# JiaweiXu8/AD-GS

Measured on AMD Instinct MI355X. Metric: fwd+bwd frames/s, higher is better.
Workload: dtype f32; 1 GPU; C3: 1000000 Gaussians, 1920x1280, SH deg 3, 8 dynamic objects, flow+semantic outputs, 1 camera/GPU/step; P=1000000, camera_pool=16 cameras / time stamps per GPU, cycled one per step (train.py:55-61), settle_steps=75, capacity_reruns=0, launch=eager, parallelism=single GPU, gradient_exchange=none, camera_streams=1

## Files before the change

ad-gs_amd/csrc/api.hip:

```cpp
#include "common.h"
#include "kernels.h"
#include "../../include/adgs_rasterizer.h"
#include "../../include/adgs_optim.h"

#include <atomic>
#include <chrono>
#include <mutex>
#include <vector>
#include <cstdlib>
#include <algorithm>
#include <cmath>
#include <cstring>

namespace adgs {

static thread_local std::string g_last_error;
struct FrameContext {
	adgs_frame_stats stats;
	size_t hint_cells, hint_fine;
	unsigned hint_max_cell_chunks;
	bool bucket_frame_pending;
	long long reruns;
	int last_order_hint;
	uint32_t* slab_bounds;
// ... 36 lines not shown
constexpr size_t IMG_HEADER_WORDS = 16;
struct ImgState {
	uint32_t* header; uint32_t* n_contrib; uint2* ranges;
	static ImgState carve(char* chunk, size_t npix, size_t ntiles, size_t* bytes) {
		Carver c(chunk); ImgState s;
		s.header = c.take<uint32_t>(IMG_HEADER_WORDS);
		s.n_contrib = c.take<uint32_t>(npix);
		s.ranges = c.take<uint2>(ntiles);
		if (bytes) *bytes = c.size();
		return s;
	}
};
struct BinState {
	uint64_t* keys_unsorted; uint64_t* keys; uint32_t* list_unsorted; uint32_t* list; char* sort_temp;
	static BinState carve(char* chunk, size_t R, size_t* bytes) {
		Carver c(chunk); BinState b;
		b.list = c.take<uint32_t>(R);
		b.list_unsorted = c.take<uint32_t>(R);
		b.keys = c.take<uint64_t>(R);
		b.keys_unsorted = c.take<uint64_t>(R);
		b.sort_temp = c.take<char>(sort_temp_bytes(R));
		if (bytes) *bytes = c.size();
		return b;
	}
};

struct GeomStateV2 {
	Splat* splats; uint8_t* clamped; uint32_t* cells_touched; uint32_t* offsets; uint32_t* fine_touched; uint4* dupinfo;
	float* gacc; float* sh0; char* scan_temp; unsigned long long* fine_total;
	float* ddir;
	uint32_t* counters; uint32_t* cell_start; uint2* cell_work; uint32_t* bounds; uint32_t* counts;
	static constexpr size_t COUNTER_WORDS = MAX_CELLS + 2 * SCAN_AUX_SLOTS + 8;
	uint32_t* cell_count() const { return counters; }
	unsigned long long* bucket_fine_total() const { return reinterpret_cast<unsigned long long*>(counters + MAX_CELLS); }
	uint32_t* d_counts() const { return counters + MAX_CELLS + 2 * SCAN_AUX_SLOTS; }
	static GeomStateV2 carve(char* chunk, size_t P, size_t* bytes, bool with_ddir, size_t ncells = 0) {
		Carver c(chunk); GeomStateV2 g;
		g.counters = c.take<uint32_t>(COUNTER_WORDS);
		g.cell_start = c.take<uint32_t>(MAX_CELLS + 1);
		g.cell_work = c.take<uint2>(MAX_CELLS + 1);
		g.splats = c.take<Splat>(P);
		g.gacc = c.take<float>(P * GACC_STRIDE);
		g.dupinfo = c.take<uint4>(P);
		g.clamped = c.take<uint8_t>(P);
		g.cells_touched = c.take<uint32_t>(P + 1);
		g.offsets = c.take<uint32_t>(P + 1);
		g.fine_touched = c.take<uint32_t>(P + 1);
		g.sh0 = c.take<float>(P * 3);
		g.fine_total = c.take<unsigned long long>(SCAN_AUX_SLOTS);
		g.scan_temp = c.take<char>(scan_temp_bytes(P + 1));
		g.ddir = with_ddir ? c.take<float>(P * 9) : nullptr;
		const size_t nc = std::min<size_t>(ncells, (size_t)MAX_CELLS + 1);
		g.bounds = c.take<uint32_t>(nc * SLAB_ROW);
		g.counts = c.take<uint32_t>(((P + 255) / 256) * nc);
		if (bytes) *bytes = c.size();
		return g;
	}
};
struct ImgStateV2 {
	uint32_t* header; uint32_t* n_contrib; uint2* cell_ranges; uint32_t* tile_last_chunk; uint32_t* tile_consumed; uint32_t* tile_order; uint32_t* tile_scanned; uint32_t* tile_batches;
	static ImgStateV2 carve(char* chunk, size_t npix, size_t ntiles, size_t ncells, size_t* bytes) {
		Carver c(chunk); ImgStateV2 s;
		s.header = c.take<uint32_t>(IMG_HEADER_WORDS);
		s.n_contrib = c.take<uint32_t>(npix);
		s.cell_ranges = c.take<uint2>(ncells);
		s.tile_last_chunk = c.take<uint32_t>(ntiles);
		s.tile_consumed = c.take<uint32_t>(ntiles);
		s.tile_order = c.take<uint32_t>(ntiles);
		s.tile_scanned = c.take<uint32_t>(ntiles);
		s.tile_batches = c.take<uint32_t>(ntiles);
		if (bytes) *bytes = c.size();
		return s;
	}
};
struct BinStateV2 {
	uint32_t* pool_cursor; uint32_t* pool;
	uint64_t* keys_unsorted; uint64_t* keys; uint32_t* list_unsorted; uint32_t* list; char* sort_temp;
	uint32_t* rec_key; uint2* rec_im; uint2* entries; uint32_t* slow_list;
	static size_t slab_grid(size_t R_cells, size_t ncells) { return std::max<size_t>(2 * R_cells / SLAB_TARGET_FOREIGN + ncells + 1, ncells << forced_lg()); }
	static int forced_lg() { const char* v = getenv("ADGS_SLABS_LG"); return (v && *v) ? std::min(std::max(atoi(v), 0), (int)MAX_SLAB_LG) : 0; }
	static size_t pool_chunks(size_t R_fine, size_t ntiles) { return R_fine / WAVE + (2 * (size_t)POOL_BLOCK + 1) * ntiles + 1; }
	static BinStateV2 carve_buckets(char* chunk, size_t R_cells, size_t R_fine, size_t ntiles, size_t* bytes, size_t ncells = 0) {
		Carver c(chunk); BinStateV2 b;
		b.pool_cursor = c.take<uint32_t>(64);
		b.pool = c.take<uint32_t>(pool_chunks(R_fine, ntiles) * CHUNK_WORDS);
		b.entries = c.take<uint2>(R_cells + 1);
		b.rec_im = c.take<uint2>(R_cells);
		b.rec_key = c.take<uint32_t>(R_cells);
		b.slow_list = c.take<uint32_t>(1 + slab_grid(R_cells, ncells));
		b.keys = nullptr; b.keys_unsorted = nullptr; b.sort_temp = nullptr; b.list = nullptr; b.list_unsorted = nullptr;
		if (bytes) *bytes = c.size();
		return b;
	}
	static BinStateV2 carve(char* chunk, size_t R_cells, size_t R_fine, size_t ntiles, size_t* bytes) {
		Carver c(chunk); BinStateV2 b;
		b.pool_cursor = c.take<uint32_t>(64);
		b.pool = c.take<uint32_t>(pool_chunks(R_fine, ntiles) * CHUNK_WORDS);
		b.list = c.take<uint32_t>(R_cells);
		b.list_unsorted = c.take<uint32_t>(R_cells);
		b.keys = c.take<uint64_t>(R_cells);
		b.keys_unsorted = c.take<uint64_t>(R_cells);
		b.sort_temp = c.take<char>(sort_temp_bytes(R_cells));
		b.rec_key = nullptr; b.rec_im = nullptr; b.entries = nullptr; b.slow_list = nullptr;
		if (bytes) *bytes = c.size();
		return b;
	}
};
// ... 1193 lines not shown
```

ad-gs_amd/csrc/binning.hip:

```cpp
#include "common.h"
#include "kernels.h"

namespace adgs {
namespace {

constexpr int CS_THREADS = MAX_CELLS;
constexpr int GS_THREADS = 512, GS_WAVES = GS_THREADS / WAVE, GS_ITEMS = GS_NMAX / GS_THREADS;

__device__ __forceinline__ uint32_t wave_incl_scan_u32(uint32_t v, int lane) {
#pragma unroll
	for (int off = 1; off < WAVE; off <<= 1) { const uint32_t o = __shfl_up(v, off, WAVE); if (lane >= off) v += o; }
	return v;
}

__device__ __forceinline__ uint32_t block_excl_scan_1024(uint32_t v, uint32_t* s_wave , uint32_t* total) {
	const int tid = threadIdx.x, lane = tid & (WAVE - 1), wid = tid / WAVE;
	const uint32_t incl = wave_incl_scan_u32(v, lane);
	__syncthreads();
	if (lane == WAVE - 1) s_wave[wid] = incl;
	__syncthreads();
	uint32_t off = 0, tot = 0;
#pragma unroll
	for (int w = 0; w < CS_THREADS / WAVE; w++) { const uint32_t x = s_wave[w]; if (w < wid) off += x; tot += x; }
	*total = tot;
	return off + incl - v;
}

__global__ void __launch_bounds__(256) bin_prepare_kernel(FramePrologue p) { run_frame_prologue(p); }

__global__ void __launch_bounds__(256) cell_colscan_kernel(uint32_t* __restrict__ counts, int nblocks, int ncells, uint32_t* __restrict__ cell_count) {
	__shared__ uint32_t s_w[256 / WAVE];
	__shared__ uint32_t s_carry;
	const int c = blockIdx.x, tid = threadIdx.x, lane = tid & (WAVE - 1), wid = tid / WAVE;
	if (tid == 0) s_carry = 0u;
	__syncthreads();
	for (int b0 = 0; b0 < nblocks; b0 += 256 * 8) {
		uint32_t v[8], sum = 0;
#pragma unroll
		for (int k = 0; k < 8; k++) v[k] = counts[(size_t)min(b0 + tid * 8 + k, nblocks - 1) * ncells + c];
#pragma unroll
		for (int k = 0; k < 8; k++) { if (b0 + tid * 8 + k >= nblocks) v[k] = 0u; sum += v[k]; }
		const uint32_t incl = wave_incl_scan_u32(sum, lane);
		if (lane == WAVE - 1) s_w[wid] = incl;
		__syncthreads();
		uint32_t off = s_carry, tot = 0;
#pragma unroll
		for (int w = 0; w < 256 / WAVE; w++) { const uint32_t x = s_w[w]; if (w < wid) off += x; tot += x; }
		uint32_t run = off + incl - sum;
#pragma unroll
		for (int k = 0; k < 8; k++) { const int b = b0 + tid * 8 + k; if (b < nblocks) counts[(size_t)b * ncells + c] = run; run += v[k]; }
		__syncthreads();
		if (tid == 0) s_carry += tot;
		__syncthreads();
	}
	if (tid == 0) cell_count[c] = s_carry;
}

__global__ void __launch_bounds__(CS_THREADS) cell_scan_kernel(CellScanArgs a) {
	__shared__ uint32_t s_wave[CS_THREADS / WAVE];
	const int c = threadIdx.x;
	uint32_t n = 0;
	if (c < a.ncells) n = a.cell_count[c];
	uint32_t total, nchunks_total, work_total;
	const uint32_t start = block_excl_scan_1024(n, s_wave, &total);
	const uint32_t nch = (n + GS_NMAX - 1) / GS_NMAX;
	(void)block_excl_scan_1024(nch, s_wave, &nchunks_total);
	uint32_t lg = 0;
	while (lg < (uint32_t)MAX_SLAB_LG && (n >> lg) > a.slab_target) lg++;
	if (a.force_lg >= 0) lg = min((uint32_t)a.force_lg, (uint32_t)MAX_SLAB_LG);
	const uint32_t m = (c < a.ncells && n) ? 1u << lg : 0u;
	const uint32_t w0 = block_excl_scan_1024(m, s_wave, &work_total);
	if (c < a.ncells) { a.cell_start[c] = start; a.cell_ranges[c] = make_uint2(start, start + n); a.cell_work[c] = make_uint2(w0, lg); }
	if (c == 0) {
		a.cell_start[a.ncells] = total; a.cell_work[a.ncells] = make_uint2(work_total, 0u);
		const uint32_t over = nchunks_total > a.max_chunks ? 1u : 0u;
		unsigned long long fine = 0ull;
		for (int k = 0; k < SCAN_AUX_SLOTS; k++) fine += a.fine_total[k];
		const uint32_t nofit = (over || total > a.cap_cells || fine > a.cap_fine) ? 1u : 0u;
		a.d_counts[0] = total; a.d_counts[1] = work_total; a.d_counts[2] = over; a.d_counts[3] = nofit;
		a.d_counts[4] = 0u; a.d_counts[5] = 0u;
		a.d_counts[6] = (uint32_t)fine; a.d_counts[7] = (uint32_t)(fine >> 32);
		if (a.box) {
			a.box->r_cells = total; a.box->r_fine = fine; a.box->oversize = over; a.box->n_groups = nchunks_total; a.box->overflow = nofit;
			if (nofit) a.box->overflow_count = a.box->overflow_count + 1u;
			a.box->cap_cells = a.cap_cells; a.box->cap_fine = a.cap_fine;
			__threadfence_system();
			a.box->seq = a.seq;
		}
	}
}

__global__ void __launch_bounds__(256) cell_scatter_kernel(int P, const uint4* __restrict__ dupinfo, const uint32_t* __restrict__ cell_start,
	const uint32_t* __restrict__ counts, uint32_t* __restrict__ rec_key, uint2* __restrict__ rec_im, uint32_t cap, int cell_tiles, int cgx, int ncells, uint32_t* __restrict__ pool_cursor, uint32_t* __restrict__ slow_list) {
	__shared__ uint32_t s_cnt[MAX_CELLS];
	__shared__ uint32_t s_base[MAX_CELLS];
	const int idx = blockIdx.x * blockDim.x + threadIdx.x;
	if (idx == 0) { *pool_cursor = 0u; slow_list[0] = 0u; }
	const uint4 d = dupinfo[min(idx, P - 1)];
	for (int c = threadIdx.x; c < ncells; c += 256) { s_cnt[c] = 0u; s_base[c] = cell_start[c] + counts[(size_t)blockIdx.x * ncells + c]; }
	__syncthreads();
	if (idx >= P) return;
	const uint32_t minx = d.x & 0xFFFFu, miny = d.x >> 16, maxx = d.y & 0xFFFFu, maxy = d.y >> 16;
	if (maxx <= minx || maxy <= miny) return;
	const uint32_t c0x = minx / cell_tiles, c1x = (maxx - 1) / cell_tiles, c0y = miny / cell_tiles, c1y = (maxy - 1) / cell_tiles;
	for (uint32_t y = c0y; y <= c1y; y++)
		for (uint32_t x = c0x; x <= c1x; x++) {
			const uint32_t c = y * cgx + x;
			const uint32_t pos = s_base[c] + atomicAdd(s_cnt + c, 1u);
			const uint32_t ty0 = y * cell_tiles, tx0 = x * cell_tiles;
			const uint32_t r0 = max(miny, ty0) - ty0, r1 = min(maxy, ty0 + cell_tiles) - ty0;
			const uint32_t q0 = max(minx, tx0) - tx0, q1 = min(maxx, tx0 + cell_tiles) - tx0;
			const uint32_t rows = ((1u << r1) - 1u) & ~((1u << r0) - 1u), cols = ((1u << q1) - 1u) & ~((1u << q0) - 1u);
			if (pos < cap) { rec_key[pos] = d.z; rec_im[pos] = make_uint2((uint32_t)idx, rows | (cols << cell_tiles)); }
		}
}

__device__ __forceinline__ uint32_t slab128_of(const uint32_t* row , uint32_t key) {
	const uint32_t q = (row[31] <= key ? 1u : 0u) + (row[63] <= key ? 1u : 0u) + (row[95] <= key ? 1u : 0u);
	uint32_t r = 0;
#pragma unroll
	for (int i = 0; i < 8; i++) {
		const uint4 v = *reinterpret_cast<const uint4*>(row + 32 * q + 4 * i);
		r += (v.x <= key ? 1u : 0u) + (v.y <= key ? 1u : 0u) + (v.z <= key ? 1u : 0u) + ((i < 7 && v.w <= key) ? 1u : 0u);
	}
	return 32u * q + r;
}

__device__ __forceinline__ void publish_bound(uint32_t* __restrict__ bounds_out, uint32_t cell, uint32_t r, uint32_t n, uint32_t key) {
	const uint32_t j = (uint32_t)(((unsigned long long)r * (unsigned)SLAB_ROW + n - 1ull) / n);
	if (j >= 1u && j < (uint32_t)SLAB_ROW && (uint32_t)(((unsigned long long)j * n) / (unsigned)SLAB_ROW) == r) bounds_out[(size_t)cell * SLAB_ROW + j - 1u] = key;
}

struct SlabLds {
	uint32_t a[GS_NMAX];
	uint32_t b[GS_NMAX];
	uint32_t c[GS_NMAX];
	uint32_t cc[256];
	uint32_t red[3 * GS_WAVES];
	uint32_t row[SLAB_ROW];
	unsigned long long stack[72];
	uint32_t nsel, below, last;
};
static_assert(GS_WAVES * 256 <= GS_NMAX, "the radix sort's per-wave digit counters live in SlabLds::c");

constexpr int BS_NB = GS_NMAX, BS_NC = 256, BS_BMAX = 32;
__device__ __forceinline__ bool bucket_rank(SlabLds& s, uint32_t n, const uint32_t (&key)[GS_ITEMS], const uint32_t (&id)[GS_ITEMS], uint32_t (&rank)[GS_ITEMS]) {
	const int tid = threadIdx.x, lane = tid & (WAVE - 1), wid = tid / WAVE;
	uint32_t fb[GS_ITEMS], arr[GS_ITEMS];
	uint32_t kmin = 0xffffffffu, kmax = 0u;
#pragma unroll
	for (int r = 0; r < GS_ITEMS; r++) if ((uint32_t)(r * GS_THREADS + tid) < n) { kmin = min(kmin, key[r]); kmax = max(kmax, key[r]); }
	__syncthreads();
// ... 203 lines not shown
#pragma unroll
	for (int r = 0; r < GS_ITEMS; r++) {
		const uint32_t i = r * GS_THREADS + tid;
		id[r] = i; src[r] = 0u;
		key[r] = a.rec_key[range.x + min((uint32_t)(((unsigned long long)(2u * i + 1u) * n_c) / (2ull * S)), n_c - 1u)];
	}
	bool radix = false;
	if (!bucket_rank(s, S, key, id, rank)) { radix = true; radix_rank(s, S, key, id, src, rank); }
#pragma unroll
	for (int r = 0; r < GS_ITEMS; r++) {
		const bool have = radix ? rank[r] != 0xffffffffu : (uint32_t)(r * GS_THREADS + tid) < S;
		if (have) publish_bound(bounds, cell, rank[r], S, key[r]);
	}
}

__global__ void __launch_bounds__(GS_THREADS, 6) slab_sort_kernel(SlabSortArgs a) {
	__shared__ __attribute__((aligned(16))) SlabLds s;
	const int tid = threadIdx.x, lane = tid & (WAVE - 1);
	if (!(a.d_counts[2] == 0u && a.d_counts[3] == 0u && a.d_counts[0] <= a.cap) || blockIdx.x >= a.d_counts[1]) return;
	for (int i = tid; i <= a.ncells; i += GS_THREADS) {
		const uint2 cwv = a.cell_work[i], rg = a.cell_ranges[min(i, a.ncells - 1)];
		s.a[i] = cwv.x; s.b[i] = cwv.y; s.c[2 * i] = rg.x; s.c[2 * i + 1] = rg.y;
	}
	__syncthreads();
	uint32_t cell = 0;
	{
		uint32_t len = (uint32_t)a.ncells;
		uint32_t lo_i = 0;
		while (len > 0u) { const uint32_t half = len >> 1; if (s.a[lo_i + half] <= blockIdx.x) { lo_i += half + 1u; len -= half + 1u; } else len = half; }
		cell = lo_i - 1u;
	}
	const uint32_t lg = s.b[cell], slab = blockIdx.x - s.a[cell];
	const int shift = MAX_SLAB_LG - (int)lg;
	const uint2 range = make_uint2(s.c[2 * cell], s.c[2 * cell + 1]);
	__syncthreads();
	const uint32_t n_c = range.y - range.x;
	if (n_c == 0u || slab >= (1u << lg)) return;
	uint32_t lo = 0u, hi = 0u; bool open_top = true, sorted = true;
	if (lg > 0u) {
		const uint32_t* row = a.bounds + (size_t)cell * SLAB_ROW;
		const uint32_t w0 = row[min(lane, 126)], w1 = row[min(lane + 1, 126)], w2 = row[min(lane + 64, 126)], w3 = row[min(lane + 65, 126)];
		sorted = __ballot((lane < 126 && w0 > w1) || (lane + 64 < 126 && w2 > w3)) == 0ull;
		if (slab > 0u) lo = row[(slab << shift) - 1u];
		open_top = slab == (1u << lg) - 1u;
		if (!open_top) hi = row[((slab + 1u) << shift) - 1u];
	}
	if (tid == 0) { s.nsel = 0u; s.below = 0u; }
	__syncthreads();
	uint32_t my_below = 0;
	if (sorted) {
		const uint32_t off = range.x & 3u, n_el = off + n_c;
		const uint4* __restrict__ kw = reinterpret_cast<const uint4*>(a.rec_key + (range.x - off));
		const uint32_t n_w = (n_el + 3u) >> 2;
		const uint64_t lt = (lane == 0) ? 0ull : (~0ull >> (WAVE - lane));
		constexpr int SW = 8;
		for (uint32_t wbase = 0; wbase < n_w; wbase += GS_THREADS * SW) {
			uint4 kq[SW];
#pragma unroll
			for (int u = 0; u < SW; u++) kq[u] = kw[min(wbase + u * GS_THREADS + tid, n_w - 1u)];
			uint32_t selbits = 0, wave_n = 0;
#pragma unroll
			for (int u = 0; u < SW; u++) {
				const uint32_t kk[4] = { kq[u].x, kq[u].y, kq[u].z, kq[u].w };
#pragma unroll
				for (int e = 0; e < 4; e++) {
					const uint32_t el = (wbase + u * GS_THREADS + tid) * 4u + e;
					const bool have = el >= off && el < n_el, sel = have && kk[e] >= lo && (open_top || kk[e] < hi);
					my_below += (have && kk[e] < lo) ? 1u : 0u;
					selbits |= sel ? 1u << (4 * u + e) : 0u;
					wave_n += (uint32_t)__popcll(__ballot(sel));
				}
			}
			if (wave_n != 0u) {
				uint32_t at0 = 0;
				if (lane == 0) at0 = atomicAdd(&s.nsel, wave_n);
				at0 = __shfl(at0, 0, WAVE);
				uint32_t run = 0;
#pragma unroll
				for (int u = 0; u < SW; u++) {
					const uint32_t kk[4] = { kq[u].x, kq[u].y, kq[u].z, kq[u].w };
#pragma unroll
					for (int e = 0; e < 4; e++) {
						const bool sel = (selbits >> (4 * u + e)) & 1u;
						const uint64_t m = __ballot(sel);
						if (m == 0ull) continue;
						const uint32_t at = at0 + run + (uint32_t)__popcll(m & lt);
						if (sel && at < (uint32_t)GS_NMAX) { s.a[at] = kk[e]; s.b[at] = (wbase + u * GS_THREADS + tid) * 4u + e - off; }
						run += (uint32_t)__popcll(m);
					}
				}
			}
		}
#pragma unroll
		for (int off = WAVE / 2; off > 0; off >>= 1) my_below += __shfl_xor(my_below, off, WAVE);
		if (lane == 0 && my_below) atomicAdd(&s.below, my_below);
	}
	__syncthreads();
	const uint32_t nsel = s.nsel, below = s.below;
	bool slow = !sorted || nsel > (uint32_t)GS_NMAX;
	uint32_t key[GS_ITEMS], id[GS_ITEMS], msk[GS_ITEMS], rank[GS_ITEMS];
	if (!slow) {
#pragma unroll
		for (int r = 0; r < GS_ITEMS; r++) {
			const uint32_t j = r * GS_THREADS + tid;
			key[r] = 0u; id[r] = 0u; msk[r] = 0u;
			if (j < nsel) { key[r] = s.a[j]; const uint2 im = a.rec_im[range.x + s.b[j]]; id[r] = im.x; msk[r] = im.y; }
		}
		slow = !bucket_rank(s, nsel, key, id, rank);
	}
	if (slow) {
		if (tid == 0) { const uint32_t at = atomicAdd(a.slow_list, 1u); if (at < a.grid) a.slow_list[1u + at] = (cell << 8) | slab; }
		return;
	}
	if (tid == 0 && nsel) atomicMax(a.d_counts + 5, 1u);
#pragma unroll
	for (int r = 0; r < GS_ITEMS; r++) {
		if ((uint32_t)(r * GS_THREADS + tid) < nsel) {
			const uint32_t at = below + rank[r];
			a.ent_f[range.x + at] = make_uint2(id[r], msk[r]);
			if (a.bounds_out) publish_bound(a.bounds_out, cell, at, n_c, key[r]);
			if (a.bounds_out2) publish_bound(a.bounds_out2, cell, at, n_c, key[r]);
		}
	}
}

__global__ void __launch_bounds__(GS_THREADS, 4) slab_sort_slow_kernel(SlabSortArgs a) {
	__shared__ __attribute__((aligned(16))) SlabLds s;
	const int tid = threadIdx.x, lane = tid & (WAVE - 1);
	const uint32_t total = a.d_counts[0];
	const bool run = a.d_counts[2] == 0u && a.d_counts[3] == 0u && total <= a.cap;
	uint32_t max_rounds = 0;
	const uint32_t n_slow = run ? min(a.slow_list[0], a.grid) : 0u;
	for (uint32_t item = blockIdx.x; item < n_slow; item += gridDim.x) {
		__syncthreads();
		const uint32_t word = a.slow_list[1 + item], cell = word >> 8, slab = word & 255u;
		const uint32_t lg = a.cell_work[cell].y;
		const int shift = MAX_SLAB_LG - (int)lg;
		const uint2 range = a.cell_ranges[cell];
		const uint32_t n_c = range.y - range.x;
		if (n_c == 0u) continue;
		{
// ... 78 lines not shown
				const bool have = radix ? rank[r] != 0xffffffffu : (uint32_t)(r * GS_THREADS + tid) < n;
				if (have && rank[r] == (uint32_t)GS_NMAX / 2) s.stack[sp] = ((unsigned long long)key[r] << 32) | id[r];
			}
			__syncthreads();
			const unsigned long long pivot = s.stack[sp];
			__syncthreads();
			if (tid == 0) s.stack[sp + 1] = hi;
			sp += 2;
			hi = pivot; all = false;
			if (sp > 68) break;
			__syncthreads();
		}
	}
	}
	__syncthreads();
	if (tid == 0) {
		if (max_rounds) atomicMax(a.d_counts + 5, max_rounds);
		__threadfence();
		s.last = atomicAdd(a.d_counts + 4, 1u) == gridDim.x - 1u ? 1u : 0u;
	}
	__syncthreads();
	if (s.last && tid == 0 && a.box) {
		__threadfence();
		a.box->max_cell_chunks = *(volatile uint32_t*)(a.d_counts + 5);
		__threadfence_system();
	}
}

__global__ void __launch_bounds__(SLAB_ROW) bounds_from_sorted_kernel(const unsigned long long* __restrict__ keys, const uint2* __restrict__ cell_ranges, const uint32_t* __restrict__ d_total,
	uint32_t cap, uint32_t* __restrict__ bounds_out) {
	const uint32_t cell = blockIdx.x, j = threadIdx.x;
	const uint2 r = cell_ranges[cell];
	const uint32_t n = r.y - r.x;
	if (j < 1u || j >= (uint32_t)SLAB_ROW || n == 0u || r.y > cap || (d_total && r.y > *d_total)) return;
	bounds_out[(size_t)cell * SLAB_ROW + j - 1u] = (uint32_t)keys[r.x + (uint32_t)(((unsigned long long)j * n) / (unsigned)SLAB_ROW)];
}

}

int launch_bin_prepare(const FramePrologue& p, hipStream_t stream) {
	const int work = max(p.n_zero, p.n_copy);
	if (work <= 0) return 0;
	hipLaunchKernelGGL(bin_prepare_kernel, dim3(work > 2048 ? 8 : 1), dim3(256), 0, stream, p);
	ADGS_HIP_CHECK(hipGetLastError());
	return 0;
}
int launch_cell_scan(const CellScanArgs& a, hipStream_t stream) {
	hipLaunchKernelGGL(cell_scan_kernel, dim3(1), dim3(CS_THREADS), 0, stream, a);
	ADGS_HIP_CHECK(hipGetLastError());
	return 0;
}
int launch_cell_colscan(uint32_t* counts, int nblocks, int ncells, uint32_t* cell_count, hipStream_t stream) {
	if (ncells == 0) return 0;
	hipLaunchKernelGGL(cell_colscan_kernel, dim3(ncells), dim3(256), 0, stream, counts, nblocks, ncells, cell_count);
	ADGS_HIP_CHECK(hipGetLastError());
	return 0;
}
int launch_cell_scatter(int P, const uint4* dupinfo, const uint32_t* cell_start, const uint32_t* counts, uint32_t* rec_key, uint2* rec_im, uint32_t cap,
	int cell_tiles, int cgx, int ncells, uint32_t* pool_cursor, uint32_t* slow_list, hipStream_t stream) {
	if (P == 0) return 0;
	hipLaunchKernelGGL(cell_scatter_kernel, dim3((P + 255) / 256), dim3(256), 0, stream, P, dupinfo, cell_start, counts, rec_key, rec_im, cap, cell_tiles, cgx, ncells, pool_cursor, slow_list);
	ADGS_HIP_CHECK(hipGetLastError());
	return 0;
}
int launch_slab_sort(const SlabSortArgs& a, hipStream_t stream) {
	if (a.ncells <= 0) return 0;
	hipLaunchKernelGGL(slab_sort_kernel, dim3(a.grid), dim3(GS_THREADS), 0, stream, a);
	hipLaunchKernelGGL(slab_sort_slow_kernel, dim3(128), dim3(GS_THREADS), 0, stream, a);
	ADGS_HIP_CHECK(hipGetLastError());
	return 0;
}
int launch_cell_sample(const SlabSortArgs& a, uint32_t* bounds, hipStream_t stream) {
	if (a.ncells <= 0) return 0;
	hipLaunchKernelGGL(cell_sample_kernel, dim3((unsigned)a.ncells), dim3(GS_THREADS), 0, stream, a, bounds);
	ADGS_HIP_CHECK(hipGetLastError());
	return 0;
}
int launch_bounds_from_sorted(const uint64_t* keys, const uint2* cell_ranges, int ncells, const uint32_t* d_total, uint32_t cap, uint32_t* bounds_out, hipStream_t stream) {
	if (ncells <= 0 || !bounds_out) return 0;
	hipLaunchKernelGGL(bounds_from_sorted_kernel, dim3(ncells), dim3(SLAB_ROW), 0, stream, reinterpret_cast<const unsigned long long*>(keys), cell_ranges, d_total, cap, bounds_out);
	ADGS_HIP_CHECK(hipGetLastError());
	return 0;
}

}
```

ad-gs_amd/csrc/kernels.h:

```cpp
#pragma once
#include "common.h"
#include "func_eval.h"

namespace adgs {

struct PreprocessArgs {
	int P, D, M, D_S;
	const float* means3D; const float* scales; float scale_modifier; const float* rotations;
	const float* opacities; const float* shs; const float* cov3D_precomp; const float* colors_precomp;
	const float* flow_points; const float* semantic;
	const float* view; const float* proj; const float* campos;
	int W, H, gx, gy;
	float tan_fovx, tan_fovy, focal_x, focal_y;
	int inv_depth;
	int* radii; Splat* splats; float* cov3D; uint8_t* clamped; uint32_t* tiles_touched;
	int v2;
	uint32_t* fine_touched;
	uint4* dupinfo;
	int cell_tiles, cgx, cgy;
	ShSource sh_src;
	const float* sh0;
	float* gacc;
	unsigned long long* fine_total;
	uint32_t* bucket_count;
// ... 22 lines not shown
int launch_render_fwd(const RenderFwdArgs& a, hipStream_t stream);

struct RenderBwdArgs {
	const uint2* ranges; const uint32_t* point_list; const Splat* splats;
	int W, H, gx, gy, D_S;
	const float* semantic; const float* bg;
	const float* final_T; const uint32_t* n_contrib;
	const float* dL_dpix; const float* dL_dpix_depth; const float* dL_dpix_flow; const float* dL_dpix_sem; const float* dL_dpix_opacity;
	bool do_color, do_flow, do_sem, do_depth, do_opacity;
	float* dL_dmean2D;
	float* dL_dconic;
	float* dL_dopacity;
	float* dL_dcolor;
	float* dL_ddepth;
	float* dL_dflow;
	float* dL_dsem;
};
int launch_render_bwd(const RenderBwdArgs& a, hipStream_t stream);

struct PreprocessBwdArgs {
	int P, D, M;
	const float* means3D; const int* radii; const float* shs; const uint8_t* clamped;
	const float* scales; const float* rotations; float scale_modifier;
	const float* cov3D;
	const float* view; const float* proj; const float* campos;
	float focal_x, focal_y, tan_fovx, tan_fovy;
	int inv_depth;
	const float* dL_dmean2D; const float* dL_dconic; const float* dL_dcolor; const float* dL_ddepth;
	float* dL_dmean3D; float* dL_dcov3D; float* dL_dsh; float* dL_dscale; float* dL_drot;
	float* gacc; const Splat* splats; int W, H;
	ShSource sh_src; ShGradDst sh_dst;
	float* out_mean2D; float* out_conic; float* out_opacity; float* out_color; float* out_depth; float* out_flow; float* out_sem;
	float* out_mean2D_abs;
	int D_S;
	int sh_staging;
	const float* ddir;
	int antialias;
};
int launch_preprocess_bwd(const PreprocessBwdArgs& a, hipStream_t stream);

constexpr int CHUNK_WORDS = 2 + WAVE;
constexpr int CHUNK_PREV = WAVE, CHUNK_COUNT = WAVE + 1;
constexpr int POOL_BLOCK = 4;
constexpr int GACC_STRIDE = 16;
constexpr int GACC_USED = 14;

constexpr int MAX_CELLS = 1024;
constexpr int SLAB_ROW = 128;
constexpr int MAX_SLAB_LG = 7;
constexpr int SLAB_TARGET = 3072;
constexpr int SLAB_TARGET_FOREIGN = 2048;
constexpr int GS_NMAX = 4096;
constexpr int MAX_CHUNKS = 16384;
struct Mailbox { volatile uint32_t seq; uint32_t r_cells; unsigned long long r_fine; uint32_t oversize, n_groups, overflow, overflow_count, max_cell_chunks;
	uint32_t cap_cells; unsigned long long cap_fine; };
int launch_bin_prepare(const FramePrologue& p, hipStream_t stream);
struct CellScanArgs {
	const uint32_t* cell_count;
	uint32_t* cell_start;
	uint2* cell_ranges; int ncells;
	uint32_t max_chunks;
	uint2* cell_work;
	int force_lg;
	uint32_t slab_target;
	uint32_t* d_counts;
	const unsigned long long* fine_total;
	uint32_t cap_cells; unsigned long long cap_fine;
	Mailbox* box; uint32_t seq;
};
int launch_cell_scan(const CellScanArgs& a, hipStream_t stream);
int launch_cell_colscan(uint32_t* counts, int nblocks, int ncells, uint32_t* cell_count, hipStream_t stream);
int launch_cell_scatter(int P, const uint4* dupinfo, const uint32_t* cell_start, const uint32_t* counts, uint32_t* rec_key, uint2* rec_im, uint32_t cap,
	int cell_tiles, int cgx, int ncells, uint32_t* pool_cursor, uint32_t* slow_list, hipStream_t stream);
struct SlabSortArgs {
	const uint2* cell_ranges; int ncells;
	const uint2* cell_work;
	uint32_t grid;
	const uint32_t* rec_key; const uint2* rec_im;
	uint2* ent_f;
	uint32_t cap;
	const uint32_t* bounds;
	uint32_t* bounds_out;
	uint32_t* bounds_out2;
	uint32_t* slow_list;
	uint32_t* d_counts;
	Mailbox* box;
};
int launch_slab_sort(const SlabSortArgs& a, hipStream_t stream);
int launch_cell_sample(const SlabSortArgs& a, uint32_t* bounds, hipStream_t stream);
int launch_bounds_from_sorted(const uint64_t* keys, const uint2* cell_ranges, int ncells, const uint32_t* d_total, uint32_t cap, uint32_t* bounds_out, hipStream_t stream);

int launch_duplicate_cells(int P, const uint4* dupinfo, const uint32_t* offsets, uint64_t* keys, uint32_t* vals,
	uint32_t cap, int cell_tiles, int cgx, uint2* cell_ranges, int ncells, uint32_t* pool_cursor, int mask_shift, hipStream_t stream);

struct RenderV2FwdArgs {
	const uint2* cell_ranges; const uint32_t* cell_list; const Splat* splats;
	const uint64_t* cell_keys; int mask_shift;
	const uint2* cell_entries;
	int W, H, gx, gy, cell_tiles, cgx;
	int ppl;
	bool has_color, has_flow, has_sem;
	const float* bg;
	const float* bg_image;
	uint32_t* pool; uint32_t* pool_cursor; uint32_t* tile_last_chunk; uint32_t* tile_consumed; uint32_t* tile_scanned; uint32_t* tile_batches;
	float* final_T; uint32_t* n_contrib;
	float* out_color; float* out_depth; float* out_flow; float* out_semantic;
	int order_mode;
	const uint32_t* fwd_order;
	const float* fwd_view; const float* fwd_sig;
	const uint32_t* overflow_flag;
	bool publish;
};
int launch_render_fwd_v2(const RenderV2FwdArgs& a, hipStream_t stream);

struct RenderV2BwdArgs {
	const Splat* splats; const uint32_t* pool; const uint32_t* tile_last_chunk; const uint32_t* tile_consumed;
	int W, H, gx, gy, ppl;
	const float* bg; const float* final_T; const uint32_t* n_contrib;
	const float* bg_image; float* dL_dbg_image;
	const float* dL_dpix; const float* dL_dpix_depth; const float* dL_dpix_flow; const float* dL_dpix_sem; const float* dL_dpix_opacity;
	bool do_color, do_flow, do_sem, do_depth, do_opacity;
	bool absgrad;
	float* gacc;
	const uint32_t* tile_order;
// ... 36 lines not shown
```

ad-gs_amd/csrc/preprocess.hip:

```cpp
#include "common.h"
#include "kernels.h"
#include "geom.h"
#include <cstdlib>

#ifndef ADGS_PRE_STAGE_U4
#define ADGS_PRE_STAGE_U4 12
#endif
namespace adgs {

namespace {

struct M3 { float v[3][3]; };

__device__ __forceinline__ M3 m3mul(const M3& a, const M3& b) {
	M3 r;
#pragma unroll
	for (int c = 0; c < 3; c++)
#pragma unroll
		for (int rr = 0; rr < 3; rr++)
			r.v[c][rr] = a.v[0][rr] * b.v[c][0] + a.v[1][rr] * b.v[c][1] + a.v[2][rr] * b.v[c][2];
	return r;
}
__device__ __forceinline__ M3 m3t(const M3& a) {
	M3 r;
// ... 91 lines not shown
	if (a.flow_points) {
		const float* fp = rs ? pos : a.flow_points;
		in.f[0] = fp[3 * i]; in.f[1] = fp[3 * i + 1]; in.f[2] = fp[3 * i + 2];
	}
	in.sem = (a.semantic && a.D_S > 0) ? a.semantic[i * a.D_S] : 0.f;
	return in;
}

template <bool STAGED, bool AA>
__device__ __forceinline__ PreOut preprocess_one(const PreprocessArgs& a, const int idx, const float* s_sh, uint32_t* s_cell, const PreIn& in);

template <bool STAGED, bool AA>
__global__ void __launch_bounds__(256) preprocess_fwd_kernel(PreprocessArgs a) {
	extern __shared__ float s_sh[];
	__shared__ uint32_t s_cell[MAX_CELLS];
	const int idx = blockIdx.x * blockDim.x + threadIdx.x;
	if (a.bucket_count) for (int c = threadIdx.x; c < a.cgx * a.cgy; c += 256) s_cell[c] = 0u;
	if (idx == 0 && a.cfg_word) *a.cfg_word = a.cfg_value;
	PreIn in;
	if (STAGED) {
		const int tid = threadIdx.x, base = blockIdx.x * 256, nvalid = min(256, a.P - base);
		if (a.sh_src.scene_dc) {
			stage_rows<true, ADGS_PRE_STAGE_U4>(s_sh, SH_ROW_REST, SH_ROW_REST, base, nvalid, a.sh_src.Ns, a.sh_src.scene_rest, a.sh_src.obj_rest, tid, 256, [&]() { in = load_pre_in(a, idx); });
		} else {
			const float4* src = reinterpret_cast<const float4*>(a.shs + (size_t)base * SH_ROW_FULL);
			constexpr int NQ4 = SH_ROW_FULL / 4;
			const int total4 = nvalid * NQ4;
			float4 v[NQ4];
#pragma unroll
			for (int u = 0; u < NQ4; u++) v[u] = ld_stream4(src + min(tid + u * 256, total4 - 1));
			in = load_pre_in(a, idx);
#pragma unroll
			for (int u = 0; u < NQ4; u++) {
				const int q = tid + u * 256;
				if (q < total4) {
					const int g = q / NQ4, c = (q - g * NQ4) * 4;
					float* d = s_sh + g * SH_ROW_FULL_LDS + c;
					d[0] = v[u].x; d[1] = v[u].y; d[2] = v[u].z; d[3] = v[u].w;
				}
			}
		}
	}
	if (STAGED || a.bucket_count) __syncthreads();
	if (a.v2 && !a.bucket_count && idx < SCAN_AUX_SLOTS) a.fine_total[idx] = 0ull;
	PreOut o = { 0u, 0u };
	if (idx < a.P) o = preprocess_one<STAGED, AA>(a, idx, s_sh, s_cell, in);
	if (a.bucket_count) {
		__shared__ uint32_t s_red[256 / WAVE];
		uint32_t nf = o.nfine;
#pragma unroll
		for (int off = WAVE / 2; off > 0; off >>= 1) nf += __shfl_xor(nf, off, WAVE);
		if ((threadIdx.x & (WAVE - 1)) == 0) s_red[threadIdx.x / WAVE] = nf;
		__syncthreads();
		for (int c = threadIdx.x; c < a.cgx * a.cgy; c += 256) a.bucket_count[(size_t)blockIdx.x * (a.cgx * a.cgy) + c] = s_cell[c];
		if (threadIdx.x == 0) {
			uint32_t n = 0;
#pragma unroll
			for (int w = 0; w < 256 / WAVE; w++) n += s_red[w];
			if (n) atomicAdd(a.fine_total + (blockIdx.x & (SCAN_AUX_SLOTS - 1)), (unsigned long long)n);
		}
	}
}

template <bool STAGED, bool AA>
__device__ __forceinline__ PreOut preprocess_one(const PreprocessArgs& a, const int idx, const float* s_sh, uint32_t* s_cell, const PreIn& in) {
	const PreOut none = { 0u, 0u };
	if (idx == 0) {
		a.tiles_touched[a.P] = 0;
		if (a.v2) a.fine_touched[a.P] = 0;
	}
	a.radii[idx] = 0;
	a.tiles_touched[idx] = 0;
	if (a.v2) { a.dupinfo[idx] = make_uint4(0u, 0u, 0u, 0u); a.fine_touched[idx] = 0; }

	const bool rs = a.sh_src.scene_xyz != nullptr && idx < a.sh_src.Ns;
	const float* pos = rs ? a.sh_src.scene_xyz : a.means3D;
	const float px = STAGED ? in.p[0] : pos[3 * (size_t)idx], py = STAGED ? in.p[1] : pos[3 * (size_t)idx + 1], pz = STAGED ? in.p[2] : pos[3 * (size_t)idx + 2];
	const float* V = a.view; const float* PJ = a.proj;
	const float vz = V[2] * px + V[6] * py + V[10] * pz + V[14];
	if (vz <= 0.2f) return none;
	const float vx = V[0] * px + V[4] * py + V[8] * pz + V[12];
	const float vy = V[1] * px + V[5] * py + V[9] * pz + V[13];
	const float hx = PJ[0] * px + PJ[4] * py + PJ[8] * pz + PJ[12];
	const float hy = PJ[1] * px + PJ[5] * py + PJ[9] * pz + PJ[13];
	const float hw = PJ[3] * px + PJ[7] * py + PJ[11] * pz + PJ[15];
	const float p_w = 1.0f / (hw + 0.0000001f);
	const float projx = hx * p_w, projy = hy * p_w;

	float c3[6];
	float opacity_in = 0.f;
	if (a.cov3D_precomp) {
#pragma unroll
		for (int k = 0; k < 6; k++) c3[k] = a.cov3D_precomp[6 * (size_t)idx + k];
	} else {
		if (rs) {
			const SceneAct act = STAGED ? scene_activations(in.s, in.q, &in.op, (size_t)0)
			                            : scene_activations(a.sh_src.scene_scaling, a.sh_src.scene_rotation, a.sh_src.scene_opacity, (size_t)idx);
			cov3d_from_values(act.s[0], act.s[1], act.s[2], a.scale_modifier, act.q[0], act.q[1], act.q[2], act.q[3], c3);
			opacity_in = act.op;
		} else if (STAGED) {
			cov3d_from_scale_rot(in.s, a.scale_modifier, in.q, c3);
		} else {
			cov3d_from_scale_rot(a.scales + 3 * (size_t)idx, a.scale_modifier, a.rotations + 4 * (size_t)idx, c3);
		}
		if (a.cov3D) {
#pragma unroll
			for (int k = 0; k < 6; k++) a.cov3D[6 * (size_t)idx + k] = c3[k];
// ... 246 lines not shown
```

Measured before the change: 1063 frames/s.

## Transpose per-block cell counts to cell-major and use DPP wave scan in slab select

```diff
diff --git a/ad-gs_amd/csrc/api.hip b/ad-gs_amd/csrc/api.hip
--- a/ad-gs_amd/csrc/api.hip
+++ b/ad-gs_amd/csrc/api.hip
@@ -112,7 +112,7 @@
 		g.ddir = with_ddir ? c.take<float>(P * 9) : nullptr;
 		const size_t nc = std::min<size_t>(ncells, (size_t)MAX_CELLS + 1);
 		g.bounds = c.take<uint32_t>(nc * SLAB_ROW);
-		g.counts = c.take<uint32_t>(((P + 255) / 256) * nc);
+		g.counts = c.take<uint32_t>(count_row_stride((int)((P + 255) / 256)) * nc);
 		if (bytes) *bytes = c.size();
 		return g;
 	}
diff --git a/ad-gs_amd/csrc/binning.hip b/ad-gs_amd/csrc/binning.hip
--- a/ad-gs_amd/csrc/binning.hip
+++ b/ad-gs_amd/csrc/binning.hip
@@ -10,6 +10,16 @@
 __device__ __forceinline__ uint32_t wave_incl_scan_u32(uint32_t v, int lane) {
 #pragma unroll
 	for (int off = 1; off < WAVE; off <<= 1) { const uint32_t o = __shfl_up(v, off, WAVE); if (lane >= off) v += o; }
+	return v;
+}
+
+__device__ __forceinline__ uint32_t wave_incl_scan_dpp_u32(uint32_t v) {
+	v += (uint32_t)__builtin_amdgcn_update_dpp(0, (int)v, 0x111, 0xF, 0xF, false);
+	v += (uint32_t)__builtin_amdgcn_update_dpp(0, (int)v, 0x112, 0xF, 0xF, false);
+	v += (uint32_t)__builtin_amdgcn_update_dpp(0, (int)v, 0x114, 0xF, 0xF, false);
+	v += (uint32_t)__builtin_amdgcn_update_dpp(0, (int)v, 0x118, 0xF, 0xF, false);
+	v += (uint32_t)__builtin_amdgcn_update_dpp(0, (int)v, 0x142, 0xA, 0xF, false);
+	v += (uint32_t)__builtin_amdgcn_update_dpp(0, (int)v, 0x143, 0xC, 0xF, false);
 	return v;
 }
 
@@ -28,32 +38,38 @@
 
 __global__ void __launch_bounds__(256) bin_prepare_kernel(FramePrologue p) { run_frame_prologue(p); }
 
-__global__ void __launch_bounds__(256) cell_colscan_kernel(uint32_t* __restrict__ counts, int nblocks, int ncells, uint32_t* __restrict__ cell_count) {
-	__shared__ uint32_t s_w[256 / WAVE];
-	__shared__ uint32_t s_carry;
+constexpr int CQ = 4;
+__global__ void __launch_bounds__(256) cell_colscan_kernel(uint32_t* __restrict__ counts, int nblocks, uint32_t* __restrict__ cell_count) {
+	__shared__ uint32_t s_w[2][256 / WAVE];
 	const int c = blockIdx.x, tid = threadIdx.x, lane = tid & (WAVE - 1), wid = tid / WAVE;
-	if (tid == 0) s_carry = 0u;
-	__syncthreads();
-	for (int b0 = 0; b0 < nblocks; b0 += 256 * 8) {
-		uint32_t v[8], sum = 0;
-#pragma unroll
-		for (int k = 0; k < 8; k++) v[k] = counts[(size_t)min(b0 + tid * 8 + k, nblocks - 1) * ncells + c];
-#pragma unroll
-		for (int k = 0; k < 8; k++) { if (b0 + tid * 8 + k >= nblocks) v[k] = 0u; sum += v[k]; }
+	const int nq = (int)(count_row_stride(nblocks) / 4);
+	uint4* __restrict__ row = reinterpret_cast<uint4*>(counts + (size_t)c * count_row_stride(nblocks));
+	uint32_t carry = 0;
+	for (int q0 = 0, trip = 0; q0 < nq; q0 += 256 * CQ, trip ^= 1) {
+		const int q = q0 + CQ * tid;
+		uint4 v[CQ];
+#pragma unroll
+		for (int k = 0; k < CQ; k++) v[k] = row[min(q + k, nq - 1)];
+		uint32_t w[4 * CQ], sum = 0;
+#pragma unroll
+		for (int k = 0; k < CQ; k++) { w[4 * k] = v[k].x; w[4 * k + 1] = v[k].y; w[4 * k + 2] = v[k].z; w[4 * k + 3] = v[k].w; }
+#pragma unroll
+		for (int k = 0; k < 4 * CQ; k++) { if (4 * q + k >= nblocks) w[k] = 0u; sum += w[k]; }
 		const uint32_t incl = wave_incl_scan_u32(sum, lane);
-		if (lane == WAVE - 1) s_w[wid] = incl;
-		__syncthreads();
-		uint32_t off = s_carry, tot = 0;
-#pragma unroll
-		for (int w = 0; w < 256 / WAVE; w++) { const uint32_t x = s_w[w]; if (w < wid) off += x; tot += x; }
+		if (lane == WAVE - 1) s_w[trip][wid] = incl;
+		__syncthreads();
+		uint32_t off = carry;
+#pragma unroll
+		for (int i = 0; i < 256 / WAVE; i++) { const uint32_t x = s_w[trip][i]; if (i < wid) off += x; carry += x; }
 		uint32_t run = off + incl - sum;
 #pragma unroll
-		for (int k = 0; k < 8; k++) { const int b = b0 + tid * 8 + k; if (b < nblocks) counts[(size_t)b * ncells + c] = run; run += v[k]; }
-		__syncthreads();
-		if (tid == 0) s_carry += tot;
-		__syncthreads();
-	}
-	if (tid == 0) cell_count[c] = s_carry;
+		for (int k = 0; k < CQ; k++) {
+			uint4 o;
+			o.x = run; run += w[4 * k]; o.y = run; run += w[4 * k + 1]; o.z = run; run += w[4 * k + 2]; o.w = run; run += w[4 * k + 3];
+			if (q + k < nq) row[q + k] = o;
+		}
+	}
+	if (tid == 0) cell_count[c] = carry;
 }
 
 __global__ void __launch_bounds__(CS_THREADS) cell_scan_kernel(CellScanArgs a) {
@@ -97,7 +113,8 @@
 	const int idx = blockIdx.x * blockDim.x + threadIdx.x;
 	if (idx == 0) { *pool_cursor = 0u; slow_list[0] = 0u; }
 	const uint4 d = dupinfo[min(idx, P - 1)];
-	for (int c = threadIdx.x; c < ncells; c += 256) { s_cnt[c] = 0u; s_base[c] = cell_start[c] + counts[(size_t)blockIdx.x * ncells + c]; }
+	const size_t stride = count_row_stride((int)gridDim.x);
+	for (int c = threadIdx.x; c < ncells; c += 256) { s_cnt[c] = 0u; s_base[c] = cell_start[c] + counts[(size_t)c * stride + blockIdx.x]; }
 	__syncthreads();
 	if (idx >= P) return;
 	const uint32_t minx = d.x & 0xFFFFu, miny = d.x >> 16, maxx = d.y & 0xFFFFu, maxy = d.y >> 16;
@@ -407,13 +424,12 @@
 		const uint32_t off = range.x & 3u, n_el = off + n_c;
 		const uint4* __restrict__ kw = reinterpret_cast<const uint4*>(a.rec_key + (range.x - off));
 		const uint32_t n_w = (n_el + 3u) >> 2;
-		const uint64_t lt = (lane == 0) ? 0ull : (~0ull >> (WAVE - lane));
 		constexpr int SW = 8;
 		for (uint32_t wbase = 0; wbase < n_w; wbase += GS_THREADS * SW) {
 			uint4 kq[SW];
 #pragma unroll
 			for (int u = 0; u < SW; u++) kq[u] = kw[min(wbase + u * GS_THREADS + tid, n_w - 1u)];
-			uint32_t selbits = 0, wave_n = 0;
+			uint32_t selbits = 0;
 #pragma unroll
 			for (int u = 0; u < SW; u++) {
 				const uint32_t kk[4] = { kq[u].x, kq[u].y, kq[u].z, kq[u].w };
@@ -423,25 +439,24 @@
 					const bool have = el >= off && el < n_el, sel = have && kk[e] >= lo && (open_top || kk[e] < hi);
 					my_below += (have && kk[e] < lo) ? 1u : 0u;
 					selbits |= sel ? 1u << (4 * u + e) : 0u;
-					wave_n += (uint32_t)__popcll(__ballot(sel));
 				}
 			}
+			const uint32_t mine = (uint32_t)__popc(selbits), incl = wave_incl_scan_dpp_u32(mine);
+			const uint32_t wave_n = (uint32_t)__builtin_amdgcn_readlane((int)incl, WAVE - 1);
 			if (wave_n != 0u) {
-				uint32_t at0 = 0;
-				if (lane == 0) at0 = atomicAdd(&s.nsel, wave_n);
-				at0 = __shfl(at0, 0, WAVE);
-				uint32_t run = 0;
+				uint32_t at = 0;
+				if (lane == 0) at = atomicAdd(&s.nsel, wave_n);
+				at = (uint32_t)__builtin_amdgcn_readfirstlane((int)at) + incl - mine;
 #pragma unroll
 				for (int u = 0; u < SW; u++) {
+					if (((selbits >> (4 * u)) & 15u) == 0u) continue;
 					const uint32_t kk[4] = { kq[u].x, kq[u].y, kq[u].z, kq[u].w };
 #pragma unroll
 					for (int e = 0; e < 4; e++) {
-						const bool sel = (selbits >> (4 * u + e)) & 1u;
-						const uint64_t m = __ballot(sel);
-						if (m == 0ull) continue;
-						const uint32_t at = at0 + run + (uint32_t)__popcll(m & lt);
-						if (sel && at < (uint32_t)GS_NMAX) { s.a[at] = kk[e]; s.b[at] = (wbase + u * GS_THREADS + tid) * 4u + e - off; }
-						run += (uint32_t)__popcll(m);
+						if ((selbits >> (4 * u + e)) & 1u) {
+							if (at < (uint32_t)GS_NMAX) { s.a[at] = kk[e]; s.b[at] = (wbase + u * GS_THREADS + tid) * 4u + e - off; }
+							at++;
+						}
 					}
 				}
 			}
@@ -626,7 +641,7 @@
 }
 int launch_cell_colscan(uint32_t* counts, int nblocks, int ncells, uint32_t* cell_count, hipStream_t stream) {
 	if (ncells == 0) return 0;
-	hipLaunchKernelGGL(cell_colscan_kernel, dim3(ncells), dim3(256), 0, stream, counts, nblocks, ncells, cell_count);
+	hipLaunchKernelGGL(cell_colscan_kernel, dim3(ncells), dim3(256), 0, stream, counts, nblocks, cell_count);
 	ADGS_HIP_CHECK(hipGetLastError());
 	return 0;
 }
diff --git a/ad-gs_amd/csrc/kernels.h b/ad-gs_amd/csrc/kernels.h
--- a/ad-gs_amd/csrc/kernels.h
+++ b/ad-gs_amd/csrc/kernels.h
@@ -98,6 +98,7 @@
 constexpr int SLAB_TARGET_FOREIGN = 2048;
 constexpr int GS_NMAX = 4096;
 constexpr int MAX_CHUNKS = 16384;
+constexpr size_t count_row_stride(int nblocks) { return ((size_t)nblocks + 3u) & ~(size_t)3u; }
 struct Mailbox { volatile uint32_t seq; uint32_t r_cells; unsigned long long r_fine; uint32_t oversize, n_groups, overflow, overflow_count, max_cell_chunks;
 	uint32_t cap_cells; unsigned long long cap_fine; };
 int launch_bin_prepare(const FramePrologue& p, hipStream_t stream);
@@ -115,7 +116,7 @@
 	Mailbox* box; uint32_t seq;
 };
 int launch_cell_scan(const CellScanArgs& a, hipStream_t stream);
-int launch_cell_colscan(uint32_t* counts, int nblocks, int ncells, uint32_t* cell_count, hipStream_t stream);
+int launch_cell_colscan(uint32_t* counts , int nblocks, int ncells, uint32_t* cell_count, hipStream_t stream);
 int launch_cell_scatter(int P, const uint4* dupinfo, const uint32_t* cell_start, const uint32_t* counts, uint32_t* rec_key, uint2* rec_im, uint32_t cap,
 	int cell_tiles, int cgx, int ncells, uint32_t* pool_cursor, uint32_t* slow_list, hipStream_t stream);
 struct SlabSortArgs {
diff --git a/ad-gs_amd/csrc/preprocess.hip b/ad-gs_amd/csrc/preprocess.hip
--- a/ad-gs_amd/csrc/preprocess.hip
+++ b/ad-gs_amd/csrc/preprocess.hip
@@ -167,7 +167,7 @@
 		for (int off = WAVE / 2; off > 0; off >>= 1) nf += __shfl_xor(nf, off, WAVE);
 		if ((threadIdx.x & (WAVE - 1)) == 0) s_red[threadIdx.x / WAVE] = nf;
 		__syncthreads();
-		for (int c = threadIdx.x; c < a.cgx * a.cgy; c += 256) a.bucket_count[(size_t)blockIdx.x * (a.cgx * a.cgy) + c] = s_cell[c];
+		for (int c = threadIdx.x; c < a.cgx * a.cgy; c += 256) a.bucket_count[(size_t)c * count_row_stride((int)gridDim.x) + blockIdx.x] = s_cell[c];
 		if (threadIdx.x == 0) {
 			uint32_t n = 0;
 #pragma unroll
```

New measurement: 1077 frames/s (median of 6 runs). +1.3%, better.
